# matinraayai/ir2rgb

Measured on AMD Instinct MI355X. Metric: generator+discriminator frames/sec at 512x1024, higher is better.
Workload: dtype bf16; 1 GPU; vid2vid training window 512x1024: 2-scale generator (composite ngf128 @256x512 + composite-local ngf64 @512x1024, tG=3) + FlowNet2 reference flow + image D (num_D=2) + 2 temporal D, 3 backward passes + Adam; batch 1 frame per GPU; parallelism=dp1 (frame-parallel sequences, RCCL gradient all-reduce)

## Files before the change

### ir2rgb_amd/csrc/adam.h

```cpp
#pragma once
#include "common.h"

#define ADAM_CHUNK 8192

struct AdamTensor {
    float *p;
    const float *g;
    float *m;
    float *v;
    long n;
};

struct AdamCoef {
    float step_size, beta1, beta2, omb1, omb2, bc2_sqrt, eps;
};

static __host__ __device__ inline AdamCoef adam_coef(float lr, float beta1, float beta2, float eps, int step) {
    const double bc1 = 1.0 - pow((double)beta1, (double)step), bc2 = 1.0 - pow((double)beta2, (double)step);
    AdamCoef k;
    k.step_size = (float)((double)lr / bc1);
    k.beta1 = beta1;
    k.beta2 = beta2;
    k.omb1 = (float)(1.0 - (double)beta1);
    k.omb2 = (float)(1.0 - (double)beta2);
    k.bc2_sqrt = (float)sqrt(bc2);
    k.eps = eps;
    return k;
}

#ifdef __HIPCC__
template <bool FUSED_M>
__device__ __forceinline__ void adam_one(float &p, float g, float &m, float &v, const AdamCoef &k) {
#pragma clang fp contract(off)
    const float step_size = k.step_size, bc2_sqrt = k.bc2_sqrt, eps = k.eps;
    const float bm = k.beta1 * m, og = k.omb1 * g;
    m = FUSED_M ? __builtin_fmaf(k.omb1, g, bm) : bm + og;
    const float o2g = k.omb2 * g, bv = k.beta2 * v;
    v = __builtin_fmaf(g, o2g, bv);
    const float denom = sqrtf(v) / bc2_sqrt + eps;
    p = __builtin_fmaf(-step_size, m / denom, p);
}

template <bool SCALED>
__device__ __forceinline__ void adam_block(const AdamTensor *__restrict__ table, const int2 *__restrict__ blocks,
                                           const AdamCoef &k, const float inv_scale) {
    const int2 tb = blocks[blockIdx.x];
    const AdamTensor t = table[tb.x];
    const long e0 = (long)tb.y * ADAM_CHUNK;
    const long e1 = min(t.n, e0 + ADAM_CHUNK);
    const bool vec = ((((uintptr_t)t.p | (uintptr_t)t.g | (uintptr_t)t.m | (uintptr_t)t.v) & 15) == 0);
    if (vec && e1 - e0 == ADAM_CHUNK) {
        typedef float vf4 __attribute__((ext_vector_type(4)));
        typedef __attribute__((address_space(1))) vf4 gf4;
        gf4 *p4 = (gf4 *)(uintptr_t)t.p, *m4 = (gf4 *)(uintptr_t)t.m, *v4 = (gf4 *)(uintptr_t)t.v;
        const gf4 *g4 = (const gf4 *)(uintptr_t)t.g;
        const long q0 = (e0 >> 2) + threadIdx.x;
#pragma unroll
        for (int half = 0; half < 2; ++half) {
            vf4 P[4], G[4], M[4], V[4];
#pragma unroll
            for (int u = 0; u < 4; ++u) {
                const long q = q0 + (half * 4 + u) * 256;
                P[u] = p4[q];
                G[u] = __builtin_nontemporal_load(&g4[q]);
                M[u] = m4[q];
                V[u] = v4[q];
            }
            if constexpr (SCALED) {
#pragma unroll
                for (int u = 0; u < 4; ++u) G[u] = G[u] * inv_scale;
            }
#pragma unroll
            for (int u = 0; u < 4; ++u) {
                const long q = q0 + (half * 4 + u) * 256;
#pragma unroll
                for (int c = 0; c < 4; ++c) {
                    float pp = P[u][c], mm = M[u][c], vv = V[u][c];
                    adam_one<true>(pp, G[u][c], mm, vv, k);
                    P[u][c] = pp; M[u][c] = mm; V[u][c] = vv;
                }
                p4[q] = P[u];
                __builtin_nontemporal_store(M[u], &m4[q]);
                __builtin_nontemporal_store(V[u], &v4[q]);
            }
        }
    } else if (vec) {
        const long q1 = e1 >> 2;
        float4 *p4 = (float4 *)t.p, *m4 = (float4 *)t.m, *v4 = (float4 *)t.v;
        const float4 *g4 = (const float4 *)t.g;
#pragma unroll
        for (int half = 0; half < 2; ++half) {
            float4 P[4], G[4], M[4], V[4];
#pragma unroll
            for (int u = 0; u < 4; ++u) {
                const long q = (e0 >> 2) + (half * 4 + u) * 256 + threadIdx.x;
                if (q < q1) { P[u] = p4[q]; G[u] = g4[q]; M[u] = m4[q]; V[u] = v4[q]; }
            }
            if constexpr (SCALED) {
#pragma unroll
                for (int u = 0; u < 4; ++u) { G[u].x *= inv_scale; G[u].y *= inv_scale; G[u].z *= inv_scale; G[u].w *= inv_scale; }
            }
#pragma unroll
            for (int u = 0; u < 4; ++u) {
                const long q = (e0 >> 2) + (half * 4 + u) * 256 + threadIdx.x;
                if (q < q1) {
                    adam_one<true>(P[u].x, G[u].x, M[u].x, V[u].x, k);
                    adam_one<true>(P[u].y, G[u].y, M[u].y, V[u].y, k);
                    adam_one<true>(P[u].z, G[u].z, M[u].z, V[u].z, k);
                    adam_one<true>(P[u].w, G[u].w, M[u].w, V[u].w, k);
                    p4[q] = P[u]; m4[q] = M[u]; v4[q] = V[u];
                }
            }
        }
        for (long e = (q1 << 2) + threadIdx.x; e < e1; e += 256) {
            float p = t.p[e], m = t.m[e], v = t.v[e], g = t.g[e];
            if constexpr (SCALED) g *= inv_scale;
            adam_one<false>(p, g, m, v, k);
            t.p[e] = p; t.m[e] = m; t.v[e] = v;
        }
    } else {
        for (long e = e0 + threadIdx.x; e < e1; e += 256) {
            float p = t.p[e], m = t.m[e], v = t.v[e], g = t.g[e];
            if constexpr (SCALED) g *= inv_scale;
            adam_one<false>(p, g, m, v, k);
            t.p[e] = p; t.m[e] = m; t.v[e] = v;
        }
    }
}
#endif
```

### ir2rgb_amd/csrc/loss_scale.hip

```cpp
#include "adam.h"

static_assert(sizeof(ir2rgb_adam_state) == 48 && offsetof(ir2rgb_adam_state, grad_sumsq) == 40, "ir2rgb_adam_state layout");
static_assert(offsetof(ir2rgb_adam_state, step_size) == 4 && offsetof(ir2rgb_adam_state, found_inf) == 32 &&
              sizeof(AdamCoef) == 28, "the coefficients of ir2rgb_adam_state are an AdamCoef");
static_assert(sizeof(ir2rgb_loss_scale_state) == 16, "ir2rgb_loss_scale_state layout");

struct CheckRow {
    double sumsq;
    float nonfinite, reserved;
};
static_assert(sizeof(CheckRow) == 16, "one 16-byte load per partial row");

#define CHECK_FINISH_THREADS 1024
#define LOSS_SCALE_MAX_OPTIMIZERS 8

__device__ __forceinline__ bool nonfinite(float x) { return (__float_as_uint(x) & 0x7f800000u) == 0x7f800000u; }

__device__ __forceinline__ double wave_sum(double v) {
#pragma unroll
    for (int d = 32; d >= 1; d >>= 1) v += __shfl_down(v, d, 64);
    return v;
}

__global__ void __launch_bounds__(256)
grad_check_kernel(const AdamTensor *__restrict__ table, const int2 *__restrict__ blocks, CheckRow *__restrict__ partial) {
    const int2 tb = blocks[blockIdx.x];
    const AdamTensor t = table[tb.x];
    const long e0 = (long)tb.y * ADAM_CHUNK;
    const long e1 = min(t.n, e0 + ADAM_CHUNK);
    const bool vec = ((((uintptr_t)t.p | (uintptr_t)t.g | (uintptr_t)t.m | (uintptr_t)t.v) & 15) == 0);
    double acc = 0.0;
    bool bad = false;
    auto take = [&](float g) { bad |= nonfinite(g); acc += (double)g * (double)g; };
    if (vec && e1 - e0 == ADAM_CHUNK) {
        typedef float vf4 __attribute__((ext_vector_type(4)));
        typedef __attribute__((address_space(1))) vf4 gf4;
        const gf4 *g4 = (const gf4 *)(uintptr_t)t.g;
        const long q0 = (e0 >> 2) + threadIdx.x;
        vf4 G[8];
#pragma unroll
        for (int u = 0; u < 8; ++u) G[u] = g4[q0 + u * 256];
#pragma unroll
        for (int u = 0; u < 8; ++u)
#pragma unroll
            for (int c = 0; c < 4; ++c) take(G[u][c]);
    } else if (vec) {
        const long qb = e0 >> 2, q1 = e1 >> 2;
        const float4 *g4 = (const float4 *)t.g;
        if (q1 > qb) {
            float4 G[8];
#pragma unroll
            for (int u = 0; u < 8; ++u) G[u] = g4[min(qb + u * 256 + threadIdx.x, q1 - 1)];
#pragma unroll
            for (int u = 0; u < 8; ++u) {
                const float keep = qb + u * 256 + threadIdx.x < q1 ? 1.f : 0.f;
                take(keep != 0.f ? G[u].x : 0.f); take(keep != 0.f ? G[u].y : 0.f);
                take(keep != 0.f ? G[u].z : 0.f); take(keep != 0.f ? G[u].w : 0.f);
            }
        }
        const long e = (q1 << 2) + threadIdx.x;
        const float g = t.g[min(e, e1 - 1)];
        take(e < e1 ? g : 0.f);
    } else {
        float G[ADAM_CHUNK / 256];
#pragma unroll
        for (int u = 0; u < ADAM_CHUNK / 256; ++u) G[u] = t.g[min(e0 + u * 256 + threadIdx.x, e1 - 1)];
#pragma unroll
        for (int u = 0; u < ADAM_CHUNK / 256; ++u) take(e0 + u * 256 + threadIdx.x < e1 ? G[u] : 0.f);
    }
    __shared__ double s_sum[4];
    __shared__ int s_bad[4];
    acc = wave_sum(acc);
    const bool wave_bad = __builtin_amdgcn_ballot_w64(bad) != 0;
    if ((threadIdx.x & 63) == 0) { s_sum[threadIdx.x >> 6] = acc; s_bad[threadIdx.x >> 6] = wave_bad; }
    __syncthreads();
    if (threadIdx.x == 0) {
        CheckRow r;
        r.sumsq = ((s_sum[0] + s_sum[1]) + s_sum[2]) + s_sum[3];
        r.nonfinite = (s_bad[0] | s_bad[1] | s_bad[2] | s_bad[3]) ? 1.f : 0.f;
        r.reserved = 0.f;
        partial[blockIdx.x] = r;
    }
}

__global__ void __launch_bounds__(CHECK_FINISH_THREADS)
grad_check_finish_kernel(const CheckRow *__restrict__ partial, int nrows, ir2rgb_adam_state *__restrict__ st,
                         const ir2rgb_loss_scale_state *__restrict__ sc, float lr, float beta1, float beta2, float eps) {
    typedef unsigned uv4 __attribute__((ext_vector_type(4)));
    const uv4 *rows = (const uv4 *)partial;
    double acc = 0.0;
    bool bad = false;
    for (int base = 0; base < nrows; base += 8 * CHECK_FINISH_THREADS) {
        uv4 R[8];
#pragma unroll
        for (int u = 0; u < 8; ++u) R[u] = rows[min(base + u * CHECK_FINISH_THREADS + (int)threadIdx.x, nrows - 1)];
#pragma unroll
        for (int u = 0; u < 8; ++u) {
            const bool in = base + u * CHECK_FINISH_THREADS + (int)threadIdx.x < nrows;
            const double s = __longlong_as_double(((long long)R[u].y << 32) | (long long)R[u].x);
            acc += in ? s : 0.0;
            bad |= in && __uint_as_float(R[u].z) != 0.f;
        }
    }
    __shared__ double s_sum[CHECK_FINISH_THREADS / 64];
    __shared__ int s_bad[CHECK_FINISH_THREADS / 64];
    acc = wave_sum(acc);
    const bool wave_bad = __builtin_amdgcn_ballot_w64(bad) != 0;
    if ((threadIdx.x & 63) == 0) { s_sum[threadIdx.x >> 6] = acc; s_bad[threadIdx.x >> 6] = wave_bad; }
    __syncthreads();
    if (threadIdx.x == 0) {
        double sumsq = 0.0;
// ... 108 lines not shown
```

### ir2rgb_amd/layers.py

```python
import contextlib

import torch
import torch.nn as nn

from . import _lib
from . import conv as C
from . import streamcheck as SC

ACT_NONE, ACT_RELU, ACT_LEAKY = 0, 1, 2
_DT = C._TORCH2DT


def _require_gpu(t, what):
    if not t.is_cuda:
        raise ValueError(f"{what}: ir2rgb_amd runs on an AMD GPU only (no CPU fallback)")


def _gather(src, idx, dst):
    if SC.ENABLED:
        SC.consumed(src, "fp32 parameter"), SC.consumed(idx, "gather plan")
    _lib.launch("ir2rgb_gather_f32", src, src, idx, dst, dst.numel())
    if SC.ENABLED:
        SC.produced(dst, "rearranged fp32 weight")
    return dst


def _gather_plan(mod, tag, weight, src):
    plans = mod.__dict__.setdefault("_ir2rgb_gather", {})
    key = (src.data_ptr(), tuple(src.shape))
    hit = plans.get(tag)
    if hit is not None and hit[0] == key:
        return hit[1]
    plan = None
    n = src.numel()
    if n < (1 << 24):
        with torch.no_grad():
            r = weight(torch.arange(1, n + 1, dtype=torch.float32, device=src.device).view_as(src)).float().contiguous()
            idx = (r.round().to(torch.int32) - 1).contiguous()
            wbuf = torch.empty(r.shape, dtype=torch.float32, device=src.device)
            ref = weight(src.detach()).float().contiguous()
            if ref.shape == wbuf.shape and torch.equal(_gather(src.detach().contiguous().view(-1), idx, wbuf), ref):
                plan = (idx, wbuf)
    plans[tag] = (key, plan)
    return plan


def packed_weight(mod, desc, weight=None, tag="w", adjoint=False):
    src = mod.weight
    key = (tag, desc.dtype, src._version, src.data_ptr(), desc.Cin, desc.Cout, desc.kh, desc.kw, desc.transposed)
    cache = mod.__dict__.setdefault("_ir2rgb_packed", {})
    hit = cache.get(tag)
    if hit is not None and hit[0] == key:
        if SC.ENABLED:
            SC.consumed(hit[1], f"packed weight '{tag}'")
        return hit[1]
    plan = None
    if SC.ENABLED:
        SC.consumed(src, "fp32 parameter")
    with torch.no_grad():
        if weight is None:
            w = src.detach()
        else:
            plan = _gather_plan(mod, tag, weight, src) if src.dtype == torch.float32 and src.is_contiguous() else None
            w = _gather(src.detach().view(-1), plan[0], plan[1]) if plan is not None else weight(src.detach())
        if w.dtype != torch.float32 or not w.is_contiguous():
            w = w.float().contiguous()
        packed = C.pack_weight(desc, w, adjoint=adjoint)
    if SC.ENABLED:
        SC.produced(packed, f"packed weight '{tag}'")
    managed = (weight is None and w.data_ptr() == src.data_ptr()) or plan is not None
    cache[tag] = (key, packed, C.ConvDesc.from_buffer_copy(desc) if managed else None, bool(adjoint), w if managed else None, plan)
    global _PACK_EPOCH
    _PACK_EPOCH += 1
    return packed


_PACK_EPOCH = 0


class WeightRepacker:

    def __init__(self, modules):
        self.modules = [m for root in modules for m in root.modules() if getattr(m, "weight", None) is not None]
        self.batch, self.sig, self.entries = None, None, []

    def _collect(self):
        ent = []
        for m in self.modules:
            for tag, hit in m.__dict__.get("_ir2rgb_packed", {}).items():
                if len(hit) == 6 and hit[2] is not None and hit[0][3] == m.weight.data_ptr():
                    ent.append((m, tag, hit))
        return ent

    def run(self):
        if getattr(self, "_epoch", None) == _PACK_EPOCH and self.entries:
            ent = self.entries
            sig = self.sig
        else:
            ent = self._collect()
            self.entries, self._epoch = ent, _PACK_EPOCH
            sig = tuple((id(m), tag, hit[1].data_ptr(), hit[0][3], hit[0][1], hit[4].data_ptr()) for m, tag, hit in ent)
        if not ent:
            return 0
        if sig != self.sig:
            by_dtype = {}
            for e in ent:
                by_dtype.setdefault(e[2][0][1], []).append(e)
            self.batch = [C.PackBatch([(hit[2], hit[4], hit[1], hit[3]) for m, tag, hit in es])
                          for es in by_dtype.values()]
            self.sig = sig
        with torch.no_grad():
            for m, tag, hit in ent:
                if hit[5] is not None:
                    _gather(m.weight.detach().view(-1), hit[5][0], hit[5][1])
        if SC.ENABLED:
            for m, tag, hit in ent:
                SC.consumed(m.weight, "fp32 parameter")
        for b in self.batch:
            b.run()
        if SC.ENABLED:
            for m, tag, hit in ent:
                SC.produced(hit[1], f"packed weight '{tag}' (batched repack)")
        for m, tag, hit in ent:
            k = hit[0]
            m._ir2rgb_packed[tag] = ((k[0], k[1], m.weight._version) + tuple(k[3:]),) + tuple(hit[1:])
        return len(ent)


_STAT_UPDATES = 1


@contextlib.contextmanager
def repeated_forward(times):
    global _STAT_UPDATES
    old, _STAT_UPDATES = _STAT_UPDATES, (tuple(int(t) for t in times) if isinstance(times, (tuple, list)) else int(times))
    try:
        yield
    finally:
        _STAT_UPDATES = old


def _bn_ptrs(bn):
    hit = bn.__dict__.get("_ir2rgb_ptrs")
    w = bn.weight
    if hit is not None and hit[0] == (w.data_ptr() if w is not None else 0):
        return hit
    rm, rv = bn.running_mean, bn.running_var
    hit = (w.data_ptr() if w is not None else 0, w, bn.bias, rm, rv, rm is not None,
           0.1 if bn.momentum is None else float(bn.momentum), float(bn.eps), bool(bn.track_running_stats))
    bn.__dict__["_ir2rgb_ptrs"] = hit
    return hit


def _bn_params(bn):
    if isinstance(bn, nn.Module):
        _, w, b, rm, rv, has_rm, momentum, eps, trs = _bn_ptrs(bn)
    else:
        w, b, rm, rv, has_rm = bn.weight, bn.bias, bn.running_mean, bn.running_var, bn.running_mean is not None
        momentum, eps, trs = 0.1 if bn.momentum is None else float(bn.momentum), float(bn.eps), bn.track_running_stats
    return w, b, rm, rv, momentum, eps, bool(trs and has_rm)


def bn_frozen(bn, training):
    return (not training) and bn.track_running_stats and bn.running_mean is not None


def bn_finalize(stats, count, bn, training=True, conv_bias=None, outs=None):
    w, b, rm, rv, momentum, eps, tracks = _bn_params(bn)
    frozen = (not training) and tracks
    ch = bn.num_features
    dev = w.device if w is not None else stats.device
    rows = 0 if stats is None else stats.shape[0]
    if outs is not None:
        scale, shift, mean, invstd = outs
    else:
        scale = torch.empty(ch, dtype=torch.float32, device=dev)
        shift = torch.empty_like(scale)
        mean = torch.empty_like(scale)
        invstd = torch.empty_like(scale)
    track = training and tracks
    use_running = track or frozen
    if SC.ENABLED and use_running:
        SC.consumed(bn.running_mean, "BatchNorm running statistics")
        if track:
            SC.produced(bn.running_mean, "BatchNorm running statistics")
    _lib.launch("ir2rgb_bn_finalize_ex", scale, stats, rows, ch, int(count), w, b, conv_bias,
                rm if use_running else None, rv if use_running else None, momentum, eps, scale, shift, mean, invstd,
                _STAT_UPDATES, int(frozen))
    if track and bn.num_batches_tracked is not None:
        _PENDING_COUNTERS.append((bn.num_batches_tracked, _STAT_UPDATES))
    return scale, shift, mean, invstd


FUSED_BN_MAX_ROWS = 128


def bn_finalize_apply(stats, count, bn, y, act, res1=None, res2=None, conv_bias=None, out=None, outs=None):
    rows, _, ch = stats.shape
    n, _, h, w = y.shape
    if outs is not None:
        scale, shift, mean, invstd = outs
    else:
# ... 157 lines not shown
```

### ir2rgb_amd/optim.py

```python
import ctypes
import math

import numpy as np
import torch

from . import _lib
from . import streamcheck as SC


class FusedAdam:
    def __init__(self, params, lr=2e-4, betas=(0.5, 0.999), eps=1e-8):
        self.params = [p for p in params if p.requires_grad]
        if not self.params:
            raise ValueError("FusedAdam: no trainable parameters")
        dev = self.params[0].device
        if dev.type != "cuda":
            raise ValueError("FusedAdam: GPU parameters only (no CPU fallback)")
        for p in self.params:
            if p.dtype != torch.float32 or not p.is_contiguous() or p.device != dev:
                raise ValueError("FusedAdam: contiguous fp32 parameters on one device")
        self.param_groups = [{"params": self.params, "lr": lr, "betas": tuple(betas), "eps": eps, "weight_decay": 0,
                              "amsgrad": False}]
        self.step_count = 0
        n = sum(p.numel() for p in self.params)
        self.exp_avg = torch.zeros(n, dtype=torch.float32, device=dev)
        self.exp_avg_sq = torch.zeros(n, dtype=torch.float32, device=dev)
        lib = _lib.lib()
        chunk = lib.ir2rgb_adam_chunk_elems()
        rows = np.zeros((len(self.params), 5), dtype=np.int64)
        blocks, off = [], 0
        for i, p in enumerate(self.params):
            k = p.numel()
            rows[i] = (p.data_ptr(), 0, self.exp_avg.data_ptr() + 4 * off, self.exp_avg_sq.data_ptr() + 4 * off, k)
            blocks += [(i, c) for c in range((k + chunk - 1) // chunk)]
            off += k
        self._rows_host = [torch.from_numpy(rows.copy()).pin_memory() for _ in range(2)]
        self._rows_np = [t.numpy() for t in self._rows_host]
        self._copied = [None, None]
        self._rows_dev = torch.empty_like(self._rows_host[0], device=dev)
        self._blocks = torch.tensor(blocks, dtype=torch.int32, device=dev)
        self._ptrs = [p.data_ptr() for p in self.params]
        self.device = dev
        self._flip = 0
        self._state = self._partial = None
        self._on_device = False

    @property
    def lr(self):
        return self.param_groups[0]["lr"]

    @lr.setter
    def lr(self, value):
        self.param_groups[0]["lr"] = value

    @property
    def betas(self):
        return self.param_groups[0]["betas"]

    @property
    def eps(self):
        return self.param_groups[0]["eps"]

    def zero_grad(self, set_to_none=True):
        for p in self.params:
            if set_to_none:
                p.grad = None
            elif p.grad is not None:
                p.grad.zero_()

    def state_dict(self):
        state = {}
        self._read_step_count()
        if self.step_count:
            for i in range(len(self.params)):
                m, v = self.moments(i)
                state[i] = {"step": torch.tensor(float(self.step_count)), "exp_avg": m.clone(), "exp_avg_sq": v.clone()}
        g = {k: v for k, v in self.param_groups[0].items() if k != "params"}
        g["params"] = list(range(len(self.params)))
        return {"state": state, "param_groups": [g]}

    def load_state_dict(self, sd):
        g = sd["param_groups"][0]
        if len(g["params"]) != len(self.params):
            raise ValueError("FusedAdam.load_state_dict: parameter count differs")
        self.param_groups[0].update({k: v for k, v in g.items() if k in ("lr", "betas", "eps")})
        self.param_groups[0]["betas"] = tuple(self.param_groups[0]["betas"])
        steps = {int(s["step"]) for s in sd["state"].values()}
        if len(steps) > 1:
            raise ValueError("FusedAdam.load_state_dict: parameters with different step counts (one launch updates all)")
        self.step_count = steps.pop() if steps else 0
        self._on_device = False
        with torch.no_grad():
            if not sd["state"]:
                self.exp_avg.zero_()
                self.exp_avg_sq.zero_()
            for i, s in sd["state"].items():
                m, v = self.moments(int(i))
                m.copy_(s["exp_avg"])
                v.copy_(s["exp_avg_sq"])

    def moments(self, i):
        off = sum(p.numel() for p in self.params[:i])
        k = self.params[i].numel()
        return self.exp_avg[off:off + k].view_as(self.params[i]), self.exp_avg_sq[off:off + k].view_as(self.params[i])

    def scaled_state(self):
        if self._state is None:
            nbytes = _lib.query("ir2rgb_loss_scale_state_bytes", 0)
            assert ctypes.sizeof(_lib.AdamState) == nbytes
            self._state = torch.zeros(nbytes // 4, dtype=torch.int32, device=self.device)
            nbytes = _lib.query("ir2rgb_grad_check_partial_bytes", self._blocks.shape[0])
            self._partial = torch.zeros(nbytes // 8, dtype=torch.float64, device=self.device)
        if not self._on_device:
            st = _lib.AdamState(step=self.step_count)
            self._state.copy_(torch.frombuffer(bytearray(bytes(st)), dtype=torch.int32))
            self._on_device = True
        return self._state

    def _read_step_count(self):
        if self._on_device:
            self.step_count = int(self._state[0].item())

    def grad_stats(self):
        st = _lib.AdamState.from_buffer_copy(self.scaled_state().cpu().numpy().tobytes())
        return bool(st.found_inf), math.sqrt(st.grad_sumsq) if st.grad_sumsq >= 0 else float("nan")

    def _refresh_table(self):
        k = self._flip
        self._flip ^= 1
        if self._copied[k] is not None:
            self._copied[k].synchronize()
        rows = self._rows_np[k]
        for i, p in enumerate(self.params):
            g = p.grad
            if g is None:
                raise RuntimeError("FusedAdam.step: a parameter has no gradient (FlatGrads assigns zeros to unused ones)")
            if g.dtype != torch.float32 or not g.is_contiguous():
                g = p.grad = g.float().contiguous()
            if p.data_ptr() != self._ptrs[i]:
                raise RuntimeError("FusedAdam.step: parameter storage moved since construction")
            rows[i, 1] = g.data_ptr()
        self._rows_dev.copy_(self._rows_host[k], non_blocking=True)
        if self._copied[k] is None:
            self._copied[k] = torch.cuda.Event()
        self._copied[k].record()

    @torch.no_grad()
    def step(self, scaler=None):
        self._refresh_table()
        nblocks = self._blocks.shape[0]
        if scaler is None:
            if self._on_device:
                self._read_step_count()
                self._on_device = False
            self.step_count += 1
            _lib.launch("ir2rgb_adam_step", self.exp_avg, self._rows_dev.data_ptr(), self._blocks.data_ptr(),
                        nblocks, self.lr, self.betas[0], self.betas[1], self.eps, self.step_count)
        else:
            state = self.scaled_state()
            _lib.launch("ir2rgb_grad_check", self.exp_avg, self._rows_dev, self._blocks, nblocks, self._partial, state,
                        scaler.state, self.lr, self.betas[0], self.betas[1], self.eps)
            _lib.launch("ir2rgb_adam_step_scaled", self.exp_avg, self._rows_dev, self._blocks, nblocks, state, scaler.state)
        torch.autograd.graph.increment_version(self.params)
        if SC.ENABLED:
            for p in self.params:
                SC.produced(p, "fp32 parameter (Adam step)")


def _fp32_exact(x):
    return float(np.float32(x)) == float(x)


class LossScaler:

    def __init__(self, device, init_scale=2.0 ** 16, growth_factor=2.0, backoff_factor=0.5, growth_interval=2000):
        device = torch.device(device)
        if device.type != "cuda":
            raise ValueError("LossScaler: GPU only (no CPU fallback; loss_scale_update_reference restates the rule)")
        check_scaler_arguments(init_scale, growth_factor, backoff_factor, growth_interval)
        self.device = device
        self.growth_factor, self.backoff_factor, self.growth_interval = float(growth_factor), float(backoff_factor), int(growth_interval)
        assert ctypes.sizeof(_lib.LossScaleState) == _lib.query("ir2rgb_loss_scale_state_bytes", 1)
        self.state = torch.zeros(ctypes.sizeof(_lib.LossScaleState) // 4, dtype=torch.float32, device=device)
        self.scale_tensor = self.state[0]
        self._write(init_scale, 0, 0)
        self._tables = {}
        self._last = []

    def _write(self, scale, tracker, skipped):
        scale = float(np.float32(scale))
        st = _lib.LossScaleState(scale=scale, inv_scale=float(np.float32(1.0 / scale)), growth_tracker=tracker, skipped=skipped)
        self.state.copy_(torch.frombuffer(bytearray(bytes(st)), dtype=torch.float32))

    def _read(self):
        return _lib.LossScaleState.from_buffer_copy(self.state.cpu().numpy().tobytes())

    def register(self, optimizers):
        key = tuple(id(o) for o in optimizers)
        if key not in self._tables:
            if not 1 <= len(optimizers) <= 8:
                raise ValueError("LossScaler.update: between 1 and 8 optimizers")
            self._tables[key] = torch.tensor([o.scaled_state().data_ptr() for o in optimizers], dtype=torch.int64,
                                             device=self.device)
        return self._tables[key]

    def forget_tables(self):
        self._tables = {}
        self._last = []

    def last_optimizers(self):
        return list(self._last)

    def update(self, optimizers):
        optimizers = list(optimizers)
        table = self.register(optimizers)
        self._last = optimizers
        _lib.launch("ir2rgb_loss_scale_update", self.state, self.state, table, len(optimizers), self.growth_factor,
                    self.backoff_factor, self.growth_interval)

    def stats(self):
        st = self._read()
        return {"scale": st.scale, "skipped": st.skipped, "grad_norms": [o.grad_stats()[1] for o in self._last]}

    def state_dict(self):
        st = self._read()
        return {"scale": st.scale, "growth_tracker": st.growth_tracker, "skipped": st.skipped,
                "growth_factor": self.growth_factor, "backoff_factor": self.backoff_factor, "growth_interval": self.growth_interval}

    def load_state_dict(self, sd):
        check_scaler_arguments(sd["scale"], sd.get("growth_factor", self.growth_factor), sd.get("backoff_factor", self.backoff_factor),
                               sd.get("growth_interval", self.growth_interval))
        self.growth_factor = float(sd.get("growth_factor", self.growth_factor))
        self.backoff_factor = float(sd.get("backoff_factor", self.backoff_factor))
        self.growth_interval = int(sd.get("growth_interval", self.growth_interval))
        self._write(sd["scale"], int(sd["growth_tracker"]), int(sd.get("skipped", 0)))


def check_scaler_arguments(scale, growth_factor, backoff_factor, growth_interval):
    if isinstance(scale, bool) or not isinstance(scale, (int, float)) or not math.isfinite(scale) or scale <= 0 or \
            not math.isfinite(float(np.float32(scale))) or float(np.float32(scale)) == 0.0:
        raise ValueError(f"loss scale: a positive finite fp32 number, got {scale!r}")
    if not (growth_factor >= 1.0 and _fp32_exact(growth_factor)) or not (0.0 < backoff_factor <= 1.0 and _fp32_exact(backoff_factor)):
        raise ValueError("loss scale: growth_factor >= 1 and backoff_factor in (0, 1], both exact in fp32")
    if isinstance(growth_interval, bool) or not isinstance(growth_interval, int) or growth_interval < 0:
        raise ValueError("loss scale: growth_interval is a count of windows (0: static scale)")

# ... 54 lines not shown
```

### ir2rgb_amd/vid2vid.py

```python
import contextlib
import os

import torch
import torch.distributed as dist
import torch.nn.functional as F

from . import autograd, layers, networks
from . import conv as _conv
from . import streamcheck as SC
from .flatgrads import FlatGrads
from .flownet import FlowNet
from .frames import FrameHistory
from .losses import _SplitGroupsFn, drop_grad_dsts, fused_losses, split_groups
from .networks import SLOT_D_TEMPORAL, SLOT_FLOWNET, _Branch, side_stream
from .optim import FusedAdam, LossScaler, check_loss_scale_option, make_loss_scaler

DEFAULTS = dict(
    input_nc=3, output_nc=3, n_input_gen_frames=3, first_layer_gen_filters=128, gen_network="composite", gen_ds_layers=3,
    gen_blocks=9, n_blocks_local=3, norm="batch", n_scales_spatial=1, fg=False, no_flow=False, n_local_enhancers=1,
    feat_num=3, first_layer_dis_filters=64, num_D=2, n_layers_D=3, no_ganFeat=False, n_frames_D=3, n_scales_temporal=2,
    lr=2e-4, beta1=0.5, lambda_feat=10.0, lambda_T=10.0, lambda_F=10.0, no_first_img=False, max_frames_per_gpu=1,
    n_frames_bp=1, compute_dtype=torch.bfloat16, flownet_dtype=torch.bfloat16,
    no_vgg=True,
    shared_fake_forward=True,
# ... 460 lines not shown
            extra[s] = (fl, cf)
        return extra

    def skipped_frames(self, rb_s, extra_flows, fake_B, flow_ref, conf_ref):
        ts = self.t_scales
        fb_s = self.hist["fake"].push(fake_B)
        fl0, cf0 = self.hist["flow"].push(flow_ref), self.hist["conf"].push(conf_ref)
        fl_s, cf_s = [None] * ts, [None] * ts
        if fl0[0] is not None:
            fl_s[0], cf_s[0] = fl0[0][:, 1:], cf0[0][:, 1:]
        for s in range(1, ts):
            if s in extra_flows:
                fl_s[s], cf_s[s] = extra_flows[s]
        return rb_s, fb_s, fl_s, cf_s

    def get_losses(self, L, LT):
        mine = [getattr(d, "vecs", None) for d in [L] + list(LT)]
        if all(v is not None for v in mine) and mine[0][0] is not None:
            imgvec, dvec, gvec = mine[0]
            g_parts = [imgvec, gvec] + [m[2] for m in mine[1:]]
            loss_G = torch.cat(g_parts).sum()
            if not self.opt["no_vgg"]:
                loss_G = loss_G + L["G_VGG"]
            loss_D = dvec.sum() * 0.5
            return loss_G, loss_D, [m[1].sum() * 0.5 for m in mine[1:]]
        loss_D = (L["D_fake"] + L["D_real"]) * 0.5
        loss_G = L["G_GAN"] + L["G_GAN_Feat"] + L["G_VGG"] + L["G_Warp"] + L["F_Flow"] + L["F_Warp"] + L["W"]
        loss_D_T = []
        for lt in LT:
            loss_G = loss_G + lt["G_T_GAN"] + lt["G_T_GAN_Feat"]
            loss_D_T.append((lt["D_T_fake"] + lt["D_T_real"]) * 0.5)
        return loss_G, loss_D, loss_D_T

    def backward_passes(self, loss_G, loss_D, loss_D_T, g_inputs=None):
        self.grads_G.zero()
        self.grads_D.zero()
        for gdt in self.grads_DT:
            gdt.zero()
        shared = self.opt["shared_fake_forward"]
        d_nets = [self.netD] + self.netD_T
        if g_inputs is None and shared:
            g_inputs = self.grads_G.params
        batched = shared and self.opt["batched_D"]
        if self.loss_scaler is not None:
            k = self.loss_scaler.scale_tensor
            loss_G, loss_D, loss_D_T = loss_G * k, loss_D * k, [l * k for l in loss_D_T]
        with autograd.backward_flags([self.netD] if shared else [], autograd.SKIP_PARAM_GRADS, 2 if batched else None), \
                autograd.backward_flags(self.netD_T if shared else [], autograd.SKIP_PARAM_GRADS, 1 if batched else None):
            loss_G.backward(retain_graph=shared, inputs=g_inputs)
        self.grads_G.all_reduce_async(self.world)
        if self._early_on:
            if self._backward_done is None:
                self._backward_done = torch.cuda.Event()
            self._backward_done.record()
        with autograd.backward_flags(d_nets if shared else [], autograd.SKIP_INPUT_GRAD):
            if self.d_streams and shared and loss_D_T:
                params = list(self.grads_D.params)
                for s in range(len(loss_D_T)):
                    params += list(self.grads_DT[s].params)
                torch.autograd.backward([loss_D] + list(loss_D_T), inputs=params)
                self.grads_D.all_reduce_async(self.world)
                for s in range(len(loss_D_T)):
                    self.grads_DT[s].all_reduce_async(self.world)
            else:
                loss_D.backward(inputs=self.grads_D.params if shared else None)
                self.grads_D.all_reduce_async(self.world)
                for s, ld in enumerate(loss_D_T):
                    ld.backward(inputs=self.grads_DT[s].params if shared else None)
                    self.grads_DT[s].all_reduce_async(self.world)

    def optimizer_steps(self, n_temporal):
        scaler = self.loss_scaler
        step = (lambda o: o.step()) if scaler is None else (lambda o: o.step(scaler))
        self.grads_G.wait()
        step(self.optimizer_G)
        self.grads_D.wait()
        step(self.optimizer_D)
        for s in range(n_temporal):
            self.grads_DT[s].wait()
            step(self.optimizer_D_T[s])
        if scaler is not None:
            scaler.update([self.optimizer_G, self.optimizer_D] + self.optimizer_D_T[:n_temporal])
        if self.repacker is not None:
            self.repacker.run()

    def train_window(self, input_A, input_B):
        fake_prev_last = self.fake_B_prev
        drop_grad_dsts()
        tG = self.opt["n_input_gen_frames"]
        real_Bp_in = input_B[:, tG - 2:]
        side = self._flow_stream(input_B)
        flow_ref, conf_ref, rb_s, extra_flows = self.reference_flows(real_Bp_in[:, 1:], real_Bp_in[:, :-1], side)
        ran_on = getattr(self.flow_net, "ran_on", None)
        _conv.SIDE_BUSY = ran_on is not None
        fake_B, fake_B_raw, flow, weight, real_A, real_Bp = self.generate(input_A, input_B)
        _conv.SIDE_BUSY = False
        real_B_prev, real_B = real_Bp[:, :-1], real_Bp[:, 1:]
        if ran_on is not None:
            torch.cuda.current_stream(input_B.device).wait_stream(ran_on)
            for t in [flow_ref, conf_ref] + [x for pair in extra_flows.values() for x in pair] + [x for x in rb_s if x is not None]:
                t.record_stream(torch.cuda.current_stream(input_B.device))
        fbp = real_B_prev[:, 0:1] if fake_prev_last is None else fake_B[:, -1:].detach()
        if fake_B.size(1) > 1:
            fbp = torch.cat([fbp, fake_B[:, :-1].detach()], 1)
        flat = lambda t: t.reshape((-1,) + tuple(t.shape[2:]))
        image_args = lambda: [flat(t) for t in (real_B, fake_B, fake_B_raw, real_A, real_B_prev, fbp, flow, weight,
                                                flow_ref, conf_ref)]
        if SC.ENABLED:
            SC.consumed(flow_ref, "reference flow (FlowNet2 replay)"), SC.consumed(conf_ref, "flow confidence (FlowNet2 replay)")
        if self.d_streams:
            rb_s, fb_s, fl_s, cf_s = self.skipped_frames(rb_s, extra_flows, fake_B, flow_ref, conf_ref)
            active = [s for s in range(self.t_scales) if rb_s[s] is not None]
            LT, joins = [], []
            for s in active:
                br = _Branch(rb_s[s], fb_s[s], fl_s[s], cf_s[s], slot=SLOT_D_TEMPORAL + s, force=True)
                with br:
                    lt = self.temporal_losses(s, rb_s[s], fb_s[s], fl_s[s], cf_s[s])
                LT.append(lt)
                joins.append((br, lt))
            L = self.image_losses(*image_args())
            for br, lt in joins:
                vec = getattr(lt, "vecs", None)
                br.join(*(list(lt.values()) + ([v for v in vec if v is not None] if vec else [])))
        else:
            L = self.image_losses(*image_args())
            rb_s, fb_s, fl_s, cf_s = self.skipped_frames(rb_s, extra_flows, fake_B, flow_ref, conf_ref)
            active = [s for s in range(self.t_scales) if rb_s[s] is not None]
            LT = [self.temporal_losses(s, rb_s[s], fb_s[s], fl_s[s], cf_s[s]) for s in active]
        loss_G, loss_D, loss_D_T = self.get_losses(L, LT)
        self.backward_passes(loss_G, loss_D, loss_D_T)
        self.optimizer_steps(len(loss_D_T))
        self.last_outputs = tuple(t.detach() for t in (fake_B, fake_B_raw, flow, weight))
        out = {"G": loss_G.detach(), "D": loss_D.detach()}
        out.update({f"D_T{s}": l.detach() for s, l in enumerate(loss_D_T)})
        out.update({k: v.detach() for k, v in L.items()})
        for s, lt in zip(active, LT):
            out.update({f"{k}{s}": v.detach() for k, v in lt.items()})
        return out


def synthetic_sequence(n_frames, h, w, seed, device, channels=3):
    g = torch.Generator(device="cpu").manual_seed(seed)
    dx, dy = [int(v) for v in torch.randint(-8, 9, (2,), generator=g)]
    pad = 8 * n_frames + 8
    out = []
    for _ in range(2):
        base = torch.randn(1, channels, h + 2 * pad, w + 2 * pad, generator=g).to(device)
        base = torch.tanh(F.avg_pool2d(F.pad(base, (7, 7, 7, 7), mode="reflect"), 15, stride=1) * 6)
        frames = [base[:, :, pad + t * dy:pad + t * dy + h, pad + t * dx:pad + t * dx + w] for t in range(n_frames)]
        out.append(torch.stack(frames, 1).contiguous())
    return out[0], out[1]
```

Before: 39.67 frames/s.

## Fuse bf16 weight repacking into the fused Adam step via LDS tiles

Conv weights whose shapes qualify get the Adam kernel to write their bf16 forward and adjoint packed layouts directly. Each block updates a tile of fp32 parameters, stages the rounded values in shared memory, and scatters them into the packed buffers. The separate repack batch is then skipped for those weights, which removes a second full pass over the parameters after every optimizer step. In exchange the Adam kernel takes on shared-memory staging, extra syncs and more complex indexing, and the weight version and step bookkeeping must stay consistent or packed weights go stale.

```diff
diff --git a/ir2rgb_amd/csrc/adam.h b/ir2rgb_amd/csrc/adam.h
--- a/ir2rgb_amd/csrc/adam.h
+++ b/ir2rgb_amd/csrc/adam.h
@@ -2,6 +2,10 @@
 #include "common.h"
 
 #define ADAM_CHUNK 8192
+#define ADAM_TILE_FLAG 0x40000000
+#define ADAM_TILE_CO 32
+#define ADAM_TILE_MAX_T 9
+#define ADAM_TILE_HALFS (ADAM_TILE_CO * (64 * ADAM_TILE_MAX_T + 4))
 
 struct AdamTensor {
     float *p;
@@ -10,6 +14,12 @@
     float *v;
     long n;
 };
+
+struct AdamSink {
+    uint16_t *fwd, *adj;
+    int Cout, Cin, T, dtype;
+};
+static_assert(sizeof(AdamSink) == 32, "ir2rgb_amd/optim.py writes 32-byte sink rows");
 
 struct AdamCoef {
     float step_size, beta1, beta2, omb1, omb2, bc2_sqrt, eps;
@@ -28,103 +38,211 @@
     return k;
 }
 
+static __host__ __device__ inline void adam_tile_range(long chunk, long nchunks, long ntiles, int *lo, int *hi) {
+    *lo = (int)(chunk * ntiles / nchunks);
+    *hi = (int)((chunk + 1) * ntiles / nchunks);
+}
+
 #ifdef __HIPCC__
-template <bool FUSED_M>
-__device__ __forceinline__ void adam_one(float &p, float g, float &m, float &v, const AdamCoef &k) {
+typedef float adam_vf4 __attribute__((ext_vector_type(4)));
+typedef adam_vf4 adam_vf4u __attribute__((aligned(4)));
+typedef __attribute__((address_space(1))) adam_vf4u adam_gf4u;
+
+__device__ __forceinline__ void adam_one(float &p, float g, float &m, float &v, const AdamCoef &k, const bool fused_m) {
 #pragma clang fp contract(off)
     const float step_size = k.step_size, bc2_sqrt = k.bc2_sqrt, eps = k.eps;
     const float bm = k.beta1 * m, og = k.omb1 * g;
-    m = FUSED_M ? __builtin_fmaf(k.omb1, g, bm) : bm + og;
+    m = fused_m ? __builtin_fmaf(k.omb1, g, bm) : bm + og;
     const float o2g = k.omb2 * g, bv = k.beta2 * v;
     v = __builtin_fmaf(g, o2g, bv);
     const float denom = sqrtf(v) / bc2_sqrt + eps;
     p = __builtin_fmaf(-step_size, m / denom, p);
 }
 
+__device__ __forceinline__ void adam_four(adam_vf4 &P, const adam_vf4 &G, adam_vf4 &M, adam_vf4 &V, const AdamCoef &k,
+                                          const bool fused_m) {
+#pragma unroll
+    for (int c = 0; c < 4; ++c) {
+        float pp = P[c], mm = M[c], vv = V[c];
+        adam_one(pp, G[c], mm, vv, k, fused_m);
+        P[c] = pp; M[c] = mm; V[c] = vv;
+    }
+}
+
+template <bool SCALED>
+__device__ __forceinline__ void adam_whole_chunk(const AdamTensor &t, long e0, const AdamCoef &k, const float inv_scale,
+                                                 const bool fused_m) {
+    typedef adam_gf4u GF4;
+    GF4 *p4 = (GF4 *)(uintptr_t)(t.p + e0), *m4 = (GF4 *)(uintptr_t)(t.m + e0), *v4 = (GF4 *)(uintptr_t)(t.v + e0);
+    const GF4 *g4 = (const GF4 *)(uintptr_t)(t.g + e0);
+#pragma unroll
+    for (int half = 0; half < 2; ++half) {
+        adam_vf4 P[4], G[4], M[4], V[4];
+#pragma unroll
+        for (int u = 0; u < 4; ++u) {
+            const int q = (half * 4 + u) * 256 + threadIdx.x;
+            P[u] = p4[q];
+            G[u] = __builtin_nontemporal_load(&g4[q]);
+            M[u] = m4[q];
+            V[u] = v4[q];
+        }
+        if constexpr (SCALED) {
+#pragma unroll
+            for (int u = 0; u < 4; ++u) G[u] = G[u] * inv_scale;
+        }
+#pragma unroll
+        for (int u = 0; u < 4; ++u) {
+            const int q = (half * 4 + u) * 256 + threadIdx.x;
+            adam_four(P[u], G[u], M[u], V[u], k, fused_m);
+            p4[q] = P[u];
+            __builtin_nontemporal_store(M[u], &m4[q]);
+            __builtin_nontemporal_store(V[u], &v4[q]);
+        }
+    }
+}
+
+template <bool SCALED>
+__device__ __forceinline__ void adam_last_chunk(const AdamTensor &t, long e0, long e1, const AdamCoef &k, const float inv_scale,
+                                                const bool vec) {
+    long tail = e0;
+    if (vec) {
+        const long q1 = e1 >> 2;
+        float4 *p4 = (float4 *)t.p, *m4 = (float4 *)t.m, *v4 = (float4 *)t.v;
+        const float4 *g4 = (const float4 *)t.g;
+#pragma unroll
+        for (int half = 0; half < 2; ++half) {
+            float4 P[4], G[4], M[4], V[4];
+#pragma unroll
+            for (int u = 0; u < 4; ++u) {
+                const long q = (e0 >> 2) + (half * 4 + u) * 256 + threadIdx.x;
+                if (q < q1) { P[u] = p4[q]; G[u] = g4[q]; M[u] = m4[q]; V[u] = v4[q]; }
+            }
+            if constexpr (SCALED) {
+#pragma unroll
+                for (int u = 0; u < 4; ++u) { G[u].x *= inv_scale; G[u].y *= inv_scale; G[u].z *= inv_scale; G[u].w *= inv_scale; }
+            }
+#pragma unroll
+            for (int u = 0; u < 4; ++u) {
+                const long q = (e0 >> 2) + (half * 4 + u) * 256 + threadIdx.x;
+                if (q < q1) {
+                    adam_one(P[u].x, G[u].x, M[u].x, V[u].x, k, true);
+                    adam_one(P[u].y, G[u].y, M[u].y, V[u].y, k, true);
+                    adam_one(P[u].z, G[u].z, M[u].z, V[u].z, k, true);
+                    adam_one(P[u].w, G[u].w, M[u].w, V[u].w, k, true);
+                    p4[q] = P[u]; m4[q] = M[u]; v4[q] = V[u];
+                }
+            }
+        }
+        tail = q1 << 2;
+    }
+    for (long e = tail + threadIdx.x; e < e1; e += 256) {
+        float p = t.p[e], m = t.m[e], v = t.v[e], g = t.g[e];
+        if constexpr (SCALED) g *= inv_scale;
+        adam_one(p, g, m, v, k, false);
+        t.p[e] = p; t.m[e] = m; t.v[e] = v;
+    }
+}
+
+template <bool SCALED>
+__device__ __forceinline__ void adam_tile_chunk(const AdamTensor &t, const AdamSink &s, int chunk, const AdamCoef &k,
+                                                const float inv_scale, const bool fused_m, uint16_t *tile) {
+    const int T = s.T, Cin = s.Cin, Cout = s.Cout, dt = s.dtype;
+    const int gx = Cin / 64, gy = (Cout + ADAM_TILE_CO - 1) / ADAM_TILE_CO;
+    int lo, hi;
+    adam_tile_range(chunk, (t.n + ADAM_CHUNK - 1) / ADAM_CHUNK, (long)gx * gy, &lo, &hi);
+    const int row = 64 * T + 4;
+    const int qrow = 16 * T;
+    adam_gf4u *pg = (adam_gf4u *)(uintptr_t)t.p, *mg = (adam_gf4u *)(uintptr_t)t.m, *vg = (adam_gf4u *)(uintptr_t)t.v;
+    const adam_gf4u *gg = (const adam_gf4u *)(uintptr_t)t.g;
+    for (int ti = lo; ti < hi; ++ti) {
+        const int by = ti / gx, bx = ti - by * gx;
+        const int co0 = by * ADAM_TILE_CO, ci0 = bx * 64;
+        const int rows = min(ADAM_TILE_CO, Cout - co0);
+        const int nq = rows * qrow;
+        for (int i0 = 0; i0 < nq; i0 += 512) {
+            adam_vf4 P[2], G[2], M[2], V[2];
+            long q[2];
+            int at[2];
+#pragma unroll
+            for (int u = 0; u < 2; ++u) {
+                const int i = i0 + u * 256 + threadIdx.x;
+                const int co_l = i / qrow, qi = i - co_l * qrow;
+                q[u] = (((long)(co0 + co_l) * Cin + ci0) * T >> 2) + qi;
+                at[u] = i < nq ? co_l * row + 4 * qi : -1;
+                if (i < nq) { P[u] = pg[q[u]]; G[u] = __builtin_nontemporal_load(&gg[q[u]]); M[u] = mg[q[u]]; V[u] = vg[q[u]]; }
+            }
+            if constexpr (SCALED) {
+#pragma unroll
+                for (int u = 0; u < 2; ++u) G[u] = G[u] * inv_scale;
+            }
+#pragma unroll
+            for (int u = 0; u < 2; ++u) {
+                if (at[u] >= 0) {
+                    adam_four(P[u], G[u], M[u], V[u], k, fused_m);
+                    pg[q[u]] = P[u];
+                    __builtin_nontemporal_store(M[u], &mg[q[u]]);
+                    __builtin_nontemporal_store(V[u], &vg[q[u]]);
+                    uint2 h;
+                    h.x = (uint32_t)f2h(P[u][0], dt) | ((uint32_t)f2h(P[u][1], dt) << 16);
+                    h.y = (uint32_t)f2h(P[u][2], dt) | ((uint32_t)f2h(P[u][3], dt) << 16);
+                    *reinterpret_cast<uint2 *>(tile + at[u]) = h;
+                }
+            }
+        }
+        __syncthreads();
+        if (s.fwd) {
+            const int kch = Cin / 64;
+            for (int i = threadIdx.x; i < rows * T * 8; i += 256) {
+                const int o8 = i & 7, rt = i >> 3;
+                const int r = rt / T, tp = rt - r * T;
+                uint32_t o[4];
+#pragma unroll
+                for (int j = 0; j < 4; ++j) {
+                    const uint32_t l = tile[r * row + (o8 * 8 + 2 * j) * T + tp];
+                    const uint32_t h = tile[r * row + (o8 * 8 + 2 * j + 1) * T + tp];
+                    o[j] = l | (h << 16);
+                }
+                const long dst = (((long)(co0 + r) * kch + bx) * T + tp) * 64 + o8 * 8;
+                *reinterpret_cast<uint4 *>(s.fwd + dst) = make_uint4(o[0], o[1], o[2], o[3]);
+            }
+        }
+        if (s.adj) {
+            const int kch = Cout / 64;
+            constexpr int L = ADAM_TILE_CO / 8;
+            for (int i = threadIdx.x; i < 64 * T * L; i += 256) {
+                const int o = i % L, rt = i / L;
+                const int r = rt / T, tp = rt - r * T;
+                uint32_t w[4];
+#pragma unroll
+                for (int j = 0; j < 4; ++j) {
+                    const uint32_t l = tile[(o * 8 + 2 * j) * row + r * T + tp];
+                    const uint32_t h = tile[(o * 8 + 2 * j + 1) * row + r * T + tp];
+                    w[j] = l | (h << 16);
+                }
+                const long dst = (((long)(ci0 + r) * kch + co0 / 64) * T + (T - 1 - tp)) * 64 + (co0 % 64) + o * 8;
+                *reinterpret_cast<uint4 *>(s.adj + dst) = make_uint4(w[0], w[1], w[2], w[3]);
+            }
+        }
+        __syncthreads();
+    }
+}
+
 template <bool SCALED>
 __device__ __forceinline__ void adam_block(const AdamTensor *__restrict__ table, const int2 *__restrict__ blocks,
                                            const AdamCoef &k, const float inv_scale) {
     const int2 tb = blocks[blockIdx.x];
     const AdamTensor t = table[tb.x];
+    const bool vec = ((((uintptr_t)t.p | (uintptr_t)t.g | (uintptr_t)t.m | (uintptr_t)t.v) & 15) == 0);
+    if (tb.y & ADAM_TILE_FLAG) {
+        __shared__ uint16_t tile[ADAM_TILE_HALFS];
+        const AdamSink *sinks = (const AdamSink *)(((uintptr_t)(blocks + gridDim.x) + 15) & ~(uintptr_t)15);
+        const AdamSink s = sinks[tb.x];
+        adam_tile_chunk<SCALED>(t, s, tb.y & ~ADAM_TILE_FLAG, k, inv_scale, vec, tile);
+        return;
+    }
     const long e0 = (long)tb.y * ADAM_CHUNK;
     const long e1 = min(t.n, e0 + ADAM_CHUNK);
-    const bool vec = ((((uintptr_t)t.p | (uintptr_t)t.g | (uintptr_t)t.m | (uintptr_t)t.v) & 15) == 0);
-    if (vec && e1 - e0 == ADAM_CHUNK) {
-        typedef float vf4 __attribute__((ext_vector_type(4)));
-        typedef __attribute__((address_space(1))) vf4 gf4;
-        gf4 *p4 = (gf4 *)(uintptr_t)t.p, *m4 = (gf4 *)(uintptr_t)t.m, *v4 = (gf4 *)(uintptr_t)t.v;
-        const gf4 *g4 = (const gf4 *)(uintptr_t)t.g;
-        const long q0 = (e0 >> 2) + threadIdx.x;
-#pragma unroll
-        for (int half = 0; half < 2; ++half) {
-            vf4 P[4], G[4], M[4], V[4];
-#pragma unroll
-            for (int u = 0; u < 4; ++u) {
-                const long q = q0 + (half * 4 + u) * 256;
-                P[u] = p4[q];
-                G[u] = __builtin_nontemporal_load(&g4[q]);
-                M[u] = m4[q];
-                V[u] = v4[q];
-            }
-            if constexpr (SCALED) {
-#pragma unroll
-                for (int u = 0; u < 4; ++u) G[u] = G[u] * inv_scale;
-            }
-#pragma unroll
-            for (int u = 0; u < 4; ++u) {
-                const long q = q0 + (half * 4 + u) * 256;
-#pragma unroll
-                for (int c = 0; c < 4; ++c) {
-                    float pp = P[u][c], mm = M[u][c], vv = V[u][c];
-                    adam_one<true>(pp, G[u][c], mm, vv, k);
-                    P[u][c] = pp; M[u][c] = mm; V[u][c] = vv;
-                }
-                p4[q] = P[u];
-                __builtin_nontemporal_store(M[u], &m4[q]);
-                __builtin_nontemporal_store(V[u], &v4[q]);
-            }
-        }
-    } else if (vec) {
-        const long q1 = e1 >> 2;
-        float4 *p4 = (float4 *)t.p, *m4 = (float4 *)t.m, *v4 = (float4 *)t.v;
-        const float4 *g4 = (const float4 *)t.g;
-#pragma unroll
-        for (int half = 0; half < 2; ++half) {
-            float4 P[4], G[4], M[4], V[4];
-#pragma unroll
-            for (int u = 0; u < 4; ++u) {
-                const long q = (e0 >> 2) + (half * 4 + u) * 256 + threadIdx.x;
-                if (q < q1) { P[u] = p4[q]; G[u] = g4[q]; M[u] = m4[q]; V[u] = v4[q]; }
-            }
-            if constexpr (SCALED) {
-#pragma unroll
-                for (int u = 0; u < 4; ++u) { G[u].x *= inv_scale; G[u].y *= inv_scale; G[u].z *= inv_scale; G[u].w *= inv_scale; }
-            }
-#pragma unroll
-            for (int u = 0; u < 4; ++u) {
-                const long q = (e0 >> 2) + (half * 4 + u) * 256 + threadIdx.x;
-                if (q < q1) {
-                    adam_one<true>(P[u].x, G[u].x, M[u].x, V[u].x, k);
-                    adam_one<true>(P[u].y, G[u].y, M[u].y, V[u].y, k);
-                    adam_one<true>(P[u].z, G[u].z, M[u].z, V[u].z, k);
-                    adam_one<true>(P[u].w, G[u].w, M[u].w, V[u].w, k);
-                    p4[q] = P[u]; m4[q] = M[u]; v4[q] = V[u];
-                }
-            }
-        }
-        for (long e = (q1 << 2) + threadIdx.x; e < e1; e += 256) {
-            float p = t.p[e], m = t.m[e], v = t.v[e], g = t.g[e];
-            if constexpr (SCALED) g *= inv_scale;
-            adam_one<false>(p, g, m, v, k);
-            t.p[e] = p; t.m[e] = m; t.v[e] = v;
-        }
-    } else {
-        for (long e = e0 + threadIdx.x; e < e1; e += 256) {
-            float p = t.p[e], m = t.m[e], v = t.v[e], g = t.g[e];
-            if constexpr (SCALED) g *= inv_scale;
-            adam_one<false>(p, g, m, v, k);
-            t.p[e] = p; t.m[e] = m; t.v[e] = v;
-        }
-    }
+    if (e1 - e0 == ADAM_CHUNK) adam_whole_chunk<SCALED>(t, e0, k, inv_scale, vec);
+    else adam_last_chunk<SCALED>(t, e0, e1, k, inv_scale, vec);
 }
 #endif
diff --git a/ir2rgb_amd/csrc/loss_scale.hip b/ir2rgb_amd/csrc/loss_scale.hip
--- a/ir2rgb_amd/csrc/loss_scale.hip
+++ b/ir2rgb_amd/csrc/loss_scale.hip
@@ -26,7 +26,7 @@
 grad_check_kernel(const AdamTensor *__restrict__ table, const int2 *__restrict__ blocks, CheckRow *__restrict__ partial) {
     const int2 tb = blocks[blockIdx.x];
     const AdamTensor t = table[tb.x];
-    const long e0 = (long)tb.y * ADAM_CHUNK;
+    const long e0 = (long)(tb.y & ~ADAM_TILE_FLAG) * ADAM_CHUNK;
     const long e1 = min(t.n, e0 + ADAM_CHUNK);
     const bool vec = ((((uintptr_t)t.p | (uintptr_t)t.g | (uintptr_t)t.m | (uintptr_t)t.v) & 15) == 0);
     double acc = 0.0;
diff --git a/ir2rgb_amd/layers.py b/ir2rgb_amd/layers.py
--- a/ir2rgb_amd/layers.py
+++ b/ir2rgb_amd/layers.py
@@ -1,4 +1,5 @@
 import contextlib
+import os
 
 import torch
 import torch.nn as nn
@@ -83,6 +84,9 @@
     def __init__(self, modules):
         self.modules = [m for root in modules for m in root.modules() if getattr(m, "weight", None) is not None]
         self.batch, self.sig, self.entries = None, None, []
+        self.adam_pack = os.environ.get("IR2RGB_ADAM_PACK", "1") != "0"
+        self.rest, self.served, self._seen, self._opt_ids = [], [], {}, ()
+        self.served_total = 0
 
     def _collect(self):
         ent = []
@@ -92,7 +96,38 @@
                     ent.append((m, tag, hit))
         return ent
 
-    def run(self):
+    @staticmethod
+    def _sink_shape(m, hit):
+        w, d, packed = m.weight, hit[2], hit[1]
+        if hit[5] is not None or w.dim() != 4 or w.dtype != torch.float32 or d.transposed:
+            return False
+        co, ci, kh, kw = w.shape
+        dims = (d.Cin, d.Cout) if hit[3] else (d.Cout, d.Cin)
+        return (dims == (co, ci) and (d.kh, d.kw) == (kh, kw) and kh * kw <= 9 and ci % 64 == 0 and (not hit[3] or co % 64 == 0)
+                and packed.numel() == w.numel() and packed.data_ptr() % 16 == 0 and w.data_ptr() % 16 == 0)
+
+    def _hand_over(self, ent, fused):
+        owner = {ptr: (o, i) for o in fused for i, ptr in enumerate(o._ptrs)}
+        sinks, served, rest = {id(o): {} for o in fused}, [], []
+        for e in ent:
+            m, tag, hit = e
+            oi = owner.get(m.weight.data_ptr()) if self._sink_shape(m, hit) else None
+            slot = sinks[id(oi[0])].setdefault(oi[1], [None, None, hit[0][1]]) if oi is not None else None
+            if slot is None or slot[int(hit[3])] is not None or slot[2] != hit[0][1]:
+                rest.append(e)
+                continue
+            slot[int(hit[3])] = hit[1]
+            served.append((m, tag, hit, oi[0]))
+        for o in fused:
+            o.set_sinks({i: tuple(v) for i, v in sinks[id(o)].items()})
+        by_dtype = {}
+        for e in rest:
+            by_dtype.setdefault(e[2][0][1], []).append(e)
+        return served, [C.PackBatch([(hit[2], hit[4], hit[1], hit[3]) for m, tag, hit in es]) for es in by_dtype.values()]
+
+    def run(self, optimizers=()):
+        from .optim import FusedAdam
+        fused = [o for o in optimizers if isinstance(o, FusedAdam)] if self.adam_pack else []
         if getattr(self, "_epoch", None) == _PACK_EPOCH and self.entries:
             ent = self.entries
             sig = self.sig
@@ -102,13 +137,18 @@
             sig = tuple((id(m), tag, hit[1].data_ptr(), hit[0][3], hit[0][1], hit[4].data_ptr()) for m, tag, hit in ent)
         if not ent:
             return 0
-        if sig != self.sig:
-            by_dtype = {}
-            for e in ent:
-                by_dtype.setdefault(e[2][0][1], []).append(e)
-            self.batch = [C.PackBatch([(hit[2], hit[4], hit[1], hit[3]) for m, tag, hit in es])
-                          for es in by_dtype.values()]
-            self.sig = sig
+        opt_ids = tuple(id(o) for o in fused)
+        full = not self.served
+        if sig != self.sig or opt_ids != self._opt_ids:
+            if sig != self.sig:
+                by_dtype = {}
+                for e in ent:
+                    by_dtype.setdefault(e[2][0][1], []).append(e)
+                self.batch = [C.PackBatch([(hit[2], hit[4], hit[1], hit[3]) for m, tag, hit in es])
+                              for es in by_dtype.values()]
+            self.served, self.rest = self._hand_over(ent, fused) if fused else ([], [])
+            self.sig, self._opt_ids, self._seen = sig, opt_ids, {}
+            full = True
         with torch.no_grad():
             for m, tag, hit in ent:
                 if hit[5] is not None:
@@ -116,8 +156,14 @@
         if SC.ENABLED:
             for m, tag, hit in ent:
                 SC.consumed(m.weight, "fp32 parameter")
-        for b in self.batch:
+        if not full:
+            stepped = {id(o): o.sink_steps != self._seen.get(id(o)) for o in fused}
+            full = any(m.weight._version != m._ir2rgb_packed[tag][0][2] + stepped[id(o)] for m, tag, hit, o in self.served)
+        for o in fused:
+            self._seen[id(o)] = o.sink_steps
+        for b in (self.batch if full else self.rest):
             b.run()
+        self.served_total += 0 if full else len(self.served)
         if SC.ENABLED:
             for m, tag, hit in ent:
                 SC.produced(hit[1], f"packed weight '{tag}' (batched repack)")
diff --git a/ir2rgb_amd/optim.py b/ir2rgb_amd/optim.py
--- a/ir2rgb_amd/optim.py
+++ b/ir2rgb_amd/optim.py
@@ -6,6 +6,42 @@
 
 from . import _lib
 from . import streamcheck as SC
+
+
+ADAM_CHUNK = 8192
+ADAM_TILE_FLAG = 0x40000000
+ADAM_TILE_CO = 32
+ADAM_TILE_MAX_T = 9
+SINK_ROW_BYTES = 32
+
+
+def tile_count(cout, cin):
+    return ((cout + ADAM_TILE_CO - 1) // ADAM_TILE_CO) * (cin // 64)
+
+
+def tile_range(chunk, nchunks, ntiles):
+    return chunk * ntiles // nchunks, (chunk + 1) * ntiles // nchunks
+
+
+def build_block_table(numels, chunk=ADAM_CHUNK, sinks=None):
+    sinks = sinks or {}
+    counts = [(int(k) + chunk - 1) // chunk for k in numels]
+    nblocks = sum(counts)
+    blocks = np.zeros((nblocks, 2), dtype=np.int32)
+    at = 0
+    for i, c in enumerate(counts):
+        blocks[at:at + c, 0] = i
+        blocks[at:at + c, 1] = np.arange(c, dtype=np.int32) | (ADAM_TILE_FLAG if i in sinks else 0)
+        at += c
+    rows = np.zeros((len(counts), SINK_ROW_BYTES // 8), dtype=np.int64)
+    for i, (fwd, adj, cout, cin, taps, dtype) in sinks.items():
+        if cin % 64 or not 1 <= taps <= ADAM_TILE_MAX_T or cout * cin * taps != numels[i] or (adj and cout % 64) or \
+                (fwd | adj) % 16 or not (fwd or adj):
+            raise ValueError(f"build_block_table: tensor {i} cannot have pack sinks {(fwd, adj, cout, cin, taps, dtype)}")
+        rows[i, 0], rows[i, 1] = fwd, adj
+        rows[i, 2:].view(np.int32)[:] = (cout, cin, taps, dtype)
+    pad = (-8 * nblocks) % 16
+    return np.concatenate([blocks.view(np.uint8).reshape(-1), np.zeros(pad, dtype=np.uint8), rows.view(np.uint8).reshape(-1)]), nblocks
 
 
 class FusedAdam:
@@ -27,18 +63,24 @@
         self.exp_avg_sq = torch.zeros(n, dtype=torch.float32, device=dev)
         lib = _lib.lib()
         chunk = lib.ir2rgb_adam_chunk_elems()
+        assert chunk == ADAM_CHUNK
         rows = np.zeros((len(self.params), 5), dtype=np.int64)
-        blocks, off = [], 0
+        off = 0
         for i, p in enumerate(self.params):
             k = p.numel()
             rows[i] = (p.data_ptr(), 0, self.exp_avg.data_ptr() + 4 * off, self.exp_avg_sq.data_ptr() + 4 * off, k)
-            blocks += [(i, c) for c in range((k + chunk - 1) // chunk)]
             off += k
         self._rows_host = [torch.from_numpy(rows.copy()).pin_memory() for _ in range(2)]
         self._rows_np = [t.numpy() for t in self._rows_host]
         self._copied = [None, None]
         self._rows_dev = torch.empty_like(self._rows_host[0], device=dev)
-        self._blocks = torch.tensor(blocks, dtype=torch.int32, device=dev)
+        table, nblocks = build_block_table([p.numel() for p in self.params], chunk)
+        self._table_host = torch.from_numpy(table).pin_memory()
+        self._table_dev = self._table_host.to(dev)
+        self._table_copied = None
+        self._blocks = self._table_dev[:8 * nblocks].view(torch.int32).view(nblocks, 2)
+        self._sinks, self._sink_keep = {}, []
+        self.sink_steps = 0
         self._ptrs = [p.data_ptr() for p in self.params]
         self.device = dev
         self._flip = 0
@@ -125,6 +167,30 @@
         st = _lib.AdamState.from_buffer_copy(self.scaled_state().cpu().numpy().tobytes())
         return bool(st.found_inf), math.sqrt(st.grad_sumsq) if st.grad_sumsq >= 0 else float("nan")
 
+    def set_sinks(self, sinks):
+        desc, keep = {}, []
+        for i, (fwd, adj, dtype) in sinks.items():
+            p = self.params[i]
+            if p.dim() != 4:
+                raise ValueError("FusedAdam.set_sinks: a convolution weight [Cout, Cin, kh, kw]")
+            for t in (fwd, adj):
+                if t is not None and (t.numel() != p.numel() or t.element_size() != 2 or t.device != p.device or not t.is_contiguous()):
+                    raise ValueError("FusedAdam.set_sinks: a packed buffer of the weight's size in a 2-byte type")
+            desc[i] = (fwd.data_ptr() if fwd is not None else 0, adj.data_ptr() if adj is not None else 0, p.shape[0], p.shape[1],
+                       p.shape[2] * p.shape[3], int(dtype))
+            keep += [fwd, adj]
+        if desc == self._sinks:
+            return
+        table, _ = build_block_table([p.numel() for p in self.params], ADAM_CHUNK, desc)
+        if self._table_copied is not None:
+            self._table_copied.synchronize()
+        self._table_host.numpy()[:] = table
+        self._table_dev.copy_(self._table_host, non_blocking=True)
+        if self._table_copied is None:
+            self._table_copied = torch.cuda.Event()
+        self._table_copied.record()
+        self._sinks, self._sink_keep = desc, keep
+
     def _refresh_table(self):
         k = self._flip
         self._flip ^= 1
@@ -162,6 +228,8 @@
                         scaler.state, self.lr, self.betas[0], self.betas[1], self.eps)
             _lib.launch("ir2rgb_adam_step_scaled", self.exp_avg, self._rows_dev, self._blocks, nblocks, state, scaler.state)
         torch.autograd.graph.increment_version(self.params)
+        if self._sinks:
+            self.sink_steps += 1
         if SC.ENABLED:
             for p in self.params:
                 SC.produced(p, "fp32 parameter (Adam step)")
diff --git a/ir2rgb_amd/vid2vid.py b/ir2rgb_amd/vid2vid.py
--- a/ir2rgb_amd/vid2vid.py
+++ b/ir2rgb_amd/vid2vid.py
@@ -566,7 +566,7 @@
         if scaler is not None:
             scaler.update([self.optimizer_G, self.optimizer_D] + self.optimizer_D_T[:n_temporal])
         if self.repacker is not None:
-            self.repacker.run()
+            self.repacker.run([self.optimizer_G, self.optimizer_D] + self.optimizer_D_T)
 
     def train_window(self, input_A, input_B):
         fake_prev_last = self.fake_B_prev
```

New measurement: 39.83 frames/s (median of 6 runs). Within noise of the previous version (+0.4%).
